# Farama-Foundation/Gymnasium-Robotics

Measured on NVIDIA H100. Metric: env-steps/s, higher is better.
Workload: dtype f32

## Files before the change

### gymnasium_robotics_b200/csrc/sim_core.cuh

```cuda
#pragma once
#include "dmodel.h"

#if defined(__CUDACC__) || defined(B200_HOST_WARP)
#define B200_WARP_CODE 1
#endif
#ifdef __CUDACC__
#define HD static __device__ __forceinline__
#define HDN static __device__ __noinline__
#define STAGE static __device__ __noinline__
#define ASSUME_SHARED_PTR(p) __builtin_assume(__isShared(p))
#define ASSUME_SHARED(c) do { __builtin_assume(__isShared((c).s)); __builtin_assume(__isShared((c).mw)); __builtin_assume(__isShared((c).h)); } while (0)
#define WARP_W 32
#define SYNC() __syncwarp()
#define ALIGN() __syncthreads()
#define ALIGN_OR(p) __syncthreads_or(p)
#elif defined(B200_HOST_WARP)
#define HD static inline
#define HDN static
#define STAGE static
#define ASSUME_SHARED(c) do { } while (0)
#define ASSUME_SHARED_PTR(p) do { } while (0)
#define WARP_W 32
#define SYNC() __syncwarp()
#define ALIGN() __syncwarp()
#define ALIGN_OR(p) (__ballot_sync(0xffffffffu, (p)) != 0u)
static inline float rsqrtf(float x) { return 1.0f / sqrtf(x); }
#else
#define HD static inline
#define HDN static
#define STAGE static
#define ASSUME_SHARED(c) do { } while (0)
#define ASSUME_SHARED_PTR(p) do { } while (0)
#define WARP_W 1
#define SYNC() do { } while (0)
#define ALIGN() do { } while (0)
#define ALIGN_OR(p) (p)
static inline float rsqrtf(float x) { return 1.0f / sqrtf(x); }
#endif

#define B200_MINVAL 1e-15f
#define B200_MINIMP 0.0001f
#define B200_MAXIMP 0.9999f

struct Ctx {
  const uint32_t* mg;
  const uint32_t* mw;
  const DMHead* h;
  float* s;
  int lane;
#ifdef B200_STAGE_TIMING
  long long* tim;
#endif
};
#ifdef B200_STAGE_TIMING
enum { TM_KIN = 0, TM_COM_M, TM_COLL, TM_CONSTR, TM_SMOOTH, TM_NBEGIN, TM_NCHECK, TM_BUILDH, TM_NDIR, TM_NMOVE, TM_INTEG, TM_BARRIER, TM_OTHER, TM_MV_MULM, TM_MV_ROWS, TM_MV_LS, TM_CK_PASSF, TM_MV_UPD, TM_COUNT };
#define TIC() long long t0_ = clock64()
#define TOC(k) do { long long t1_ = clock64(); c.tim[k] += t1_ - t0_; t0_ = t1_; } while (0)
#else
#define TIC() do { } while (0)
#define TOC(k) do { } while (0)
#endif
#ifdef __CUDACC__
extern __shared__ __align__(128) uint32_t b200_smem[];
#endif
template <bool REBUILD>
HD Ctx stage_ctx(const Ctx& c) {
#ifdef __CUDACC__
  if (REBUILD) {
    uint32_t tid;
    asm volatile("mov.u32 %0, %%tid.x;" : "=r"(tid));
    Ctx r = c;
    const DMHead* h = (const DMHead*)b200_smem;
    r.s = (float*)(b200_smem + h->hot_words) + (tid >> 5) * h->scr_words;
    r.lane = (int)(tid & 31);
    return r;
  }
#endif
  return c;
}
#define MI(name) ((const int*)(c.mw + c.h->o_##name))
#define MU(name) ((const uint32_t*)(c.mw + c.h->o_##name))
#define MF(name) ((const float*)(c.mw + c.h->o_##name))
#ifdef B200_KITCHEN_GROUPS
#define PAIR_I(name) ((const int*)(c.mg + c.h->o_##name))
#define PAIR_F(name) ((const float*)(c.mg + c.h->o_##name))
#else
#define PAIR_I(name) MI(name)
#define PAIR_F(name) MF(name)
#endif
#define GI(name) ((const int*)(c.mg + c.h->o_##name))
#define GF(name) ((const float*)(c.mg + c.h->o_##name))
#define SF(name) (c.s + c.h->s_##name)
#define SI(name) ((int*)(c.s + c.h->s_##name))
#define LANES(i, n) for (int i = c.lane; i < (n); i += WARP_W)

HD float wsum(float v) {
#ifdef B200_WARP_CODE
  for (int o = 16; o; o >>= 1) v += __shfl_xor_sync(0xffffffffu, v, o);
#endif
  return v;
}
HD float wmax(float v) {
#ifdef B200_WARP_CODE
  for (int o = 16; o; o >>= 1) v = fmaxf(v, __shfl_xor_sync(0xffffffffu, v, o));
#endif
  return v;
}
HD int wsumi(int v) {
#ifdef B200_WARP_CODE
  for (int o = 16; o; o >>= 1) v += __shfl_xor_sync(0xffffffffu, v, o);
#endif
  return v;
}
HD int wexscan(int v, int lane, int* total) {
#ifdef B200_WARP_CODE
  int x = v;
  for (int o = 1; o < 32; o <<= 1) { int y = __shfl_up_sync(0xffffffffu, x, o); if (lane >= o) x += y; }
  *total = __shfl_sync(0xffffffffu, x, 31);
  return x - v;
#else
  (void)lane; *total = v; return 0;
#endif
}
HD int ffs_pop(uint32_t& m) {
#ifdef __CUDACC__
  int b = __ffs(m) - 1;
#else
  int b = __builtin_ctz(m);
#endif
  m &= m - 1;
  return b;
}
#ifdef B200_WIDE
typedef unsigned long long dmask_t;
HD int ffs_pop(dmask_t& m) {
#ifdef __CUDACC__
  int b = __ffsll((long long)m) - 1;
#else
  int b = __builtin_ctzll(m);
#endif
  m &= m - 1;
  return b;
}
// ... 1118 lines not shown
      if (id >= h->ncon_max) break;
      float* cr = SF(con) + id * CON_WORDS;
      cr[0] = o.pos[k][0]; cr[1] = o.pos[k][1]; cr[2] = o.pos[k][2];
      cr[3] = o.nrm[k][0]; cr[4] = o.nrm[k][1]; cr[5] = o.nrm[k][2];
      cr[6] = o.dist[k];
      ((int*)cr)[7] = p;
      ((int*)cr)[C_DIMGRP] = gid << 8;
      kept++;
    }
    if (ocnt > 0) {
      int* gi = (int*)(SF(group) + gid * GRP_WORDS);
      int ba = MI(geom_body)[PAIR_I(pair_geom1)[p]], bb = PAIR_I(pair_geom2)[p] < 0 ? 0 : MI(geom_body)[PAIR_I(pair_geom2)[p]];
      dmask_t ma = DM(body_ancdof, ba), mb = DM(body_ancdof, bb);
      const int bodies = GI(geom_mjb)[PAIR_I(pair_geom1)[p]] | ((PAIR_I(pair_geom2)[p] < 0 ? 0 : GI(geom_mjb)[PAIR_I(pair_geom2)[p]]) << 8);
      ((uint32_t*)gi)[G_RANGE] = (uint32_t)(basec + slot) | (uint32_t)kept << 8 | (uint32_t)bodies << 16;
      grp_set_masks(gi, ma ^ mb, mb);
    }
    if (c.lane == 0) {
      int nn = basec + total; if (nn > h->ncon_max) { nn = h->ncon_max; cnt[CNT_OVERFLOW] |= 2; }
      int ng = baseg + gtotal; if (ng > h->ngrp_max - DM_NWELD_MAX) { ng = h->ngrp_max - DM_NWELD_MAX; cnt[CNT_OVERFLOW] |= 4; }
      cnt[CNT_NCON] = nn; cnt[CNT_NGRP] = ng;
    }
    SYNC();
  }
  LANES(id, cnt[CNT_NCON]) {
    float* cr = SF(con) + id * CON_WORDS;
    const float pos[3] = {cr[0], cr[1], cr[2]}, dist = cr[6];
    float fr9[9] = {cr[3], cr[4], cr[5], 0, 0, 0, 0, 0, 0};
    const int p = ((const int*)cr)[7], gid8 = ((const int*)cr)[C_DIMGRP];
    make_frame(fr9);
    float r[3] = {pos[0] - h->ref[0], pos[1] - h->ref[1], pos[2] - h->ref[2]};
    for (int a = 0; a < 3; a++) { float* w = cr + C_W + 6 * a; cross3(w, r, fr9 + 3 * a); w[3] = fr9[3 * a]; w[4] = fr9[3 * a + 1]; w[5] = fr9[3 * a + 2]; }
    const float* fr = GF(pair_friction) + 3 * p;
    int dim = GI(pair_condim)[p];
    float mu0 = fr[0];
    cr[C_MU] = mu0; cr[C_MU + 1] = fr[1];
#ifdef B200_KITCHEN
    cr[C_MU + 2] = fr[2];
#endif
    float incl = PAIR_F(pair_margin)[p] - GF(pair_gap)[p];
    float solimp[5] = {GF(pair_solimp)[5 * p], GF(pair_solimp)[5 * p + 1], GF(pair_solimp)[5 * p + 2], GF(pair_solimp)[5 * p + 3], GF(pair_solimp)[5 * p + 4]};
    float solref[2] = {GF(pair_solref)[2 * p], GF(pair_solref)[2 * p + 1]};
    float imp = impedance(solimp, dist, incl);
    float K, Bc;
    ref_kb(c, solref, solimp[1], &K, &Bc);
    float tran = GF(pair_invweight)[2 * p];
    float R;
    if (dim == 1) R = fmaxf((1 - imp) / imp * tran, B200_MINVAL);
    else {
      float R0 = fmaxf((1 - imp) / imp * (tran + mu0 * mu0 * tran), B200_MINVAL);
      float mu = mu0 * rsqrtf(h->impratio);
      R = fmaxf(2 * mu * mu * R0, B200_MINVAL);
    }
    cr[C_D] = 1.0f / R;
    cr[C_U] = K * imp * (dist - incl); cr[C_U + 1] = 0; cr[C_U + 2] = 0; cr[C_U + 3] = 0;
#ifdef B200_KITCHEN
    cr[C_U + 4] = 0; cr[C_U + 5] = 0;
#endif
    cr[C_JV] = Bc;
    ((int*)cr)[C_DIMGRP] = dim | gid8;
    if (HF && h->nsensor > 0) {
      float* cx = SF(conx) + id * CX_WORDS;
      cx[CX_POS] = pos[0]; cx[CX_POS + 1] = pos[1]; cx[CX_POS + 2] = pos[2];
      ((int*)cx)[CX_PAIR] = p;
    }
  }
  SYNC();
}

#ifdef B200_KITCHEN
HD void con_w(const float* cr, int k, float* w) {
  if (k < 3) { const float* s = cr + C_W + 6 * k; w[0] = s[0]; w[1] = s[1]; w[2] = s[2]; w[3] = s[3]; w[4] = s[4]; w[5] = s[5]; }
  else { const float* s = cr + C_W + 6 * (k - 3) + 3; w[0] = s[0]; w[1] = s[1]; w[2] = s[2]; w[3] = w[4] = w[5] = 0; }
}
HD float con_mu(const float* cr, int k) { return k < 3 ? cr[C_MU] : (k == 3 ? cr[C_MU + 1] : cr[C_MU + 2]); }
#else
HD void con_w(const float* cr, int k, float* w) {
  if (k < 3) { const float* s = cr + C_W + 6 * k; w[0] = s[0]; w[1] = s[1]; w[2] = s[2]; w[3] = s[3]; w[4] = s[4]; w[5] = s[5]; }
  else { w[0] = cr[C_W + 3]; w[1] = cr[C_W + 4]; w[2] = cr[C_W + 5]; w[3] = w[4] = w[5] = 0; }
}
HD float con_mu(const float* cr, int k) { return k < 3 ? cr[C_MU] : cr[C_MU + 1]; }
#endif
HD int con_dim(const float* cr) { return ((const int*)cr)[C_DIMGRP] & 0xff; }
HD int con_grp(const float* cr) { return ((const int*)cr)[C_DIMGRP] >> 8; }

template <bool HF>
STAGE void make_constraint(const Ctx c) {
  ASSUME_SHARED(c);
  const DMHead* h = c.h;
  int* cnt = SI(counters);
  if (c.lane == 0) { cnt[CNT_NDR] = 0; cnt[CNT_NWELD] = 0; }
  SYNC();
  for (int e = 0; e < h->neq; e++) {
    if (!MI(eq_active)[e] || MI(eq_type)[e] != B200_EQ_WELD) continue;
    const int nw = cnt[CNT_NWELD], gid = cnt[CNT_NGRP];
    float* wr = SF(weld) + nw * WELD_WORDS;
    const float* data = MF(eq_data) + 11 * e;
    int s1 = MI(eq_obj1)[e], s2 = MI(eq_obj2)[e], b1 = 0, b2 = 0;
    float p1[3] = {0, 0, 0}, p2[3] = {0, 0, 0}, q1[4] = {1, 0, 0, 0}, q2[4] = {1, 0, 0, 0}, t[3];
    if (s1 >= 0) { b1 = MI(site_body)[s1]; qmul(q1, SF(xquat) + 4 * b1, MF(site_quat) + 4 * s1); qrot(t, SF(xquat) + 4 * b1, MF(site_pos) + 3 * s1); for (int k = 0; k < 3; k++) p1[k] = SF(xpos)[3 * b1 + k] + t[k]; }
    if (s2 >= 0) { b2 = MI(site_body)[s2]; qmul(q2, SF(xquat) + 4 * b2, MF(site_quat) + 4 * s2); qrot(t, SF(xquat) + 4 * b2, MF(site_pos) + 3 * s2); for (int k = 0; k < 3; k++) p2[k] = SF(xpos)[3 * b2 + k] + t[k]; }
    qrot(t, q1, data + 3); for (int k = 0; k < 3; k++) p1[k] += t[k];
    qrot(t, q2, data + 0); for (int k = 0; k < 3; k++) p2[k] += t[k];
    const float ts = data[10];
    float quat[4], quat1[4] = {q2[0], -q2[1], -q2[2], -q2[3]}, quat2[4];
    qmul(quat, q1, data + 6);
    qmul(quat2, quat1, quat);
    const bool use1 = b1 > 0 && DM(body_ancdof, b1) != 0;
    float r[3];
    for (int k = 0; k < 3; k++) r[k] = (use1 ? p1[k] : p2[k]) - h->ref[k];
    float K, Bc;
    ref_kb(c, MF(eq_solref) + 2 * e, MF(eq_solimp)[5 * e + 1], &K, &Bc);
    LANES(k, 6) {
      float* w = wr + W_W + 6 * k;
      float cp;
      if (k < 3) {
        float e3[3] = {k == 0 ? 1.f : 0.f, k == 1 ? 1.f : 0.f, k == 2 ? 1.f : 0.f};
        cross3(w, r, e3); w[3] = e3[0]; w[4] = e3[1]; w[5] = e3[2];
        cp = k == 0 ? p1[0] - p2[0] : (k == 1 ? p1[1] - p2[1] : p1[2] - p2[2]);
      } else {
        const int kk = k - 3;
        for (int a = 0; a < 3; a++) {
          float qa[4] = {0, a == 0 ? 1.f : 0.f, a == 1 ? 1.f : 0.f, a == 2 ? 1.f : 0.f}, t1[4], t2[4];
          qmul(t1, quat1, qa); qmul(t2, t1, quat);
          w[a] = 0.5f * ts * (kk == 0 ? t2[1] : (kk == 1 ? t2[2] : t2[3])); w[3 + a] = 0;
        }
        cp = ts * (kk == 0 ? quat2[1] : (kk == 1 ? quat2[2] : quat2[3]));
      }
      float imp = impedance(MF(eq_solimp) + 5 * e, cp, 0.f);
      float R = fmaxf((1 - imp) / imp * MF(eq_invweight)[2 * e + (k < 3 ? 0 : 1)], B200_MINVAL);
      wr[W_D + k] = 1.0f / R; wr[W_JAR + k] = K * imp * cp;
    }
    if (c.lane == 0) {
      wr[W_B] = Bc;
      ((int*)wr)[W_GRP] = gid;
      int* gi = (int*)(SF(group) + gid * GRP_WORDS);
      dmask_t ma = DM(body_ancdof, b2), mb = DM(body_ancdof, b1);
      gi[G_RANGE] = 0;
      grp_set_masks(gi, ma ^ mb, mb);
    }
    SYNC();
    if (c.lane == 0) { cnt[CNT_NGRP] = gid + 1; cnt[CNT_NWELD] = nw + 1; }
    SYNC();
  }
  for (int base = 0; base < h->njnt; base += WARP_W) {
    int j = base + c.lane;
    int nrow = 0; float dist0 = 0, dist1 = 0, sgn0 = 0, sgn1 = 0;
    if (j < h->njnt && MI(jnt_limited)[j] && MI(jnt_type)[j] != B200_JNT_FREE) {
      float q = SF(qpos)[MI(jnt_qposadr)[j]], margin = MF(jnt_margin)[j];
      float dl = q - MF(jnt_range)[2 * j], du = MF(jnt_range)[2 * j + 1] - q;
      if (dl < margin) { dist0 = dl; sgn0 = 1.f; nrow = 1; }
      if (du < margin) { if (nrow) { dist1 = du; sgn1 = -1.f; } else { dist0 = du; sgn0 = -1.f; } nrow++; }
    }
    int total, slot = wexscan(nrow, c.lane, &total);
    int basec = cnt[CNT_NDR];
    SYNC();
#pragma unroll
    for (int k = 0; k < 2; k++) {
      int id = basec + slot + k;
      if (k >= nrow || id >= h->ndr_max) continue;
      const float distk = k ? dist1 : dist0, sgnk = k ? sgn1 : sgn0;
      float* dr = SF(dofrow) + id * DR_WORDS;
      int* di = (int*)dr;
      int d = MI(jnt_dofadr)[j];
      float margin = MF(jnt_margin)[j];
      float solimp[5] = {GF(jnt_solimp)[5 * j], GF(jnt_solimp)[5 * j + 1], GF(jnt_solimp)[5 * j + 2], GF(jnt_solimp)[5 * j + 3], GF(jnt_solimp)[5 * j + 4]};
      float solref[2] = {GF(jnt_solref)[2 * j], GF(jnt_solref)[2 * j + 1]};
      float imp = impedance(solimp, distk, margin);
      float K, Bc;
      ref_kb(c, solref, solimp[1], &K, &Bc);
      float R = fmaxf((1 - imp) / imp * MF(dof_invweight0)[d], B200_MINVAL);
      di[DR_DOF] = d; dr[DR_COEF] = sgnk; di[DR_DOF2] = -1; dr[DR_COEF2] = 0;
      dr[DR_D] = 1.0f / R; dr[DR_JAR] = K * imp * (distk - margin); dr[DR_JV] = Bc;
    }
    if (c.lane == 0) { int nn = basec + total; if (nn > h->ndr_max) { nn = h->ndr_max; cnt[CNT_OVERFLOW] |= 8; } cnt[CNT_NDR] = nn; }
    SYNC();
  }
  if (HF) for (int base = 0; base < h->nten; base += WARP_W) {
    int t = base + c.lane;
    int nrow = 0; float dist0 = 0, dist1 = 0, sgn0 = 0, sgn1 = 0;
    if (t < h->nten) {
      float len = MF(ten_coef)[2 * t] * SF(qpos)[MI(ten_qadr)[2 * t]];
      if (MI(ten_dof)[2 * t + 1] >= 0) len += MF(ten_coef)[2 * t + 1] * SF(qpos)[MI(ten_qadr)[2 * t + 1]];
      float margin = MF(ten_margin)[t];
      float dl = len - MF(ten_range)[2 * t], du = MF(ten_range)[2 * t + 1] - len;
      if (dl < margin) { dist0 = dl; sgn0 = 1.f; nrow = 1; }
      if (du < margin) { if (nrow) { dist1 = du; sgn1 = -1.f; } else { dist0 = du; sgn0 = -1.f; } nrow++; }
    }
    int total, slot = wexscan(nrow, c.lane, &total);
    int basec = cnt[CNT_NDR];
    SYNC();
#pragma unroll
    for (int k = 0; k < 2; k++) {
      int id = basec + slot + k;
      if (k >= nrow || id >= h->ndr_max) continue;
      const float distk = k ? dist1 : dist0, sgnk = k ? sgn1 : sgn0;
      float* dr = SF(dofrow) + id * DR_WORDS;
      int* di = (int*)dr;
      float margin = MF(ten_margin)[t];
      float solimp[5] = {GF(ten_solimp)[5 * t], GF(ten_solimp)[5 * t + 1], GF(ten_solimp)[5 * t + 2], GF(ten_solimp)[5 * t + 3], GF(ten_solimp)[5 * t + 4]};
      float solref[2] = {GF(ten_solref)[2 * t], GF(ten_solref)[2 * t + 1]};
      float imp = impedance(solimp, distk, margin);
      float K, Bc;
      ref_kb(c, solref, solimp[1], &K, &Bc);
      float R = fmaxf((1 - imp) / imp * GF(ten_invweight)[t], B200_MINVAL);
      di[DR_DOF] = MI(ten_dof)[2 * t]; dr[DR_COEF] = sgnk * MF(ten_coef)[2 * t];
      di[DR_DOF2] = MI(ten_dof)[2 * t + 1]; dr[DR_COEF2] = sgnk * MF(ten_coef)[2 * t + 1];
      dr[DR_D] = 1.0f / R; dr[DR_JAR] = K * imp * (distk - margin); dr[DR_JV] = Bc;
    }
    if (c.lane == 0) { int nn = basec + total; if (nn > h->ndr_max) { nn = h->ndr_max; cnt[CNT_OVERFLOW] |= 8; } cnt[CNT_NDR] = nn; }
    SYNC();
  }
#ifdef B200_KITCHEN
  if (c.lane == 0) {
    for (int e = 0; e < h->neq; e++) {
      if (!MI(eq_active)[e] || MI(eq_type)[e] != B200_EQ_JOINT) continue;
      int id = cnt[CNT_NDR];
      if (id >= h->ndr_max) { cnt[CNT_OVERFLOW] |= 8; break; }
      const float* data = MF(eq_data) + 11 * e;
      int j1 = MI(eq_obj1)[e], j2 = MI(eq_obj2)[e];
      float pos = SF(qpos)[MI(jnt_qposadr)[j1]] - MF(jnt_qpos0)[j1], deriv = 0.f;
      if (j2 >= 0) {
        float dif = SF(qpos)[MI(jnt_qposadr)[j2]] - MF(jnt_qpos0)[j2];
        pos -= data[0] + dif * (data[1] + dif * (data[2] + dif * (data[3] + dif * data[4])));
        deriv = data[1] + dif * (2 * data[2] + dif * (3 * data[3] + dif * 4 * data[4]));
      } else pos -= data[0];
      float* dr = SF(dofrow) + id * DR_WORDS;
      int* di = (int*)dr;
      float imp = impedance(MF(eq_solimp) + 5 * e, pos, 0.f);
      float K, Bc;
      ref_kb(c, MF(eq_solref) + 2 * e, MF(eq_solimp)[5 * e + 1], &K, &Bc);
      float R = fmaxf((1 - imp) / imp * MF(eq_invweight)[2 * e], B200_MINVAL);
      di[DR_DOF] = MI(jnt_dofadr)[j1]; dr[DR_COEF] = 1.f;
      di[DR_DOF2] = j2 >= 0 ? MI(jnt_dofadr)[j2] : -1; dr[DR_COEF2] = -deriv;
      dr[DR_D] = -1.0f / R; dr[DR_JAR] = K * imp * pos; dr[DR_JV] = Bc;
      cnt[CNT_NDR] = id + 1;
    }
  }
  SYNC();
#endif
  if (HF) { LANES(d, h->nfric) SF(fric)[d] = 0.f; SYNC(); }
}

template <bool HF>
STAGE void rows_from_vec(const Ctx c, const float* vec) {
  ASSUME_SHARED(c);
  ASSUME_SHARED_PTR(vec);
  const int* cnt = SI(counters);
  int ngrp = cnt[CNT_NGRP];
  LANES(idx, ngrp * 6) {
    int g = idx / 6, a = idx - 6 * g;
    float* gr = SF(group) + g * GRP_WORDS;
    dmask_t S = grp_mask(gr), sg = grp_sign(gr);
    float acc = 0;
    while (S) { int j = ffs_pop(S); float t = SF(cdof)[6 * j + a] * vec[j]; acc += DBIT(sg, j) ? t : -t; }
    gr[G_V + a] = acc;
  }
  SYNC();
  LANES(i, cnt[CNT_NCON]) {
    float* cr = SF(con) + i * CON_WORDS;
    int dim = con_dim(cr), nbase = dim == 1 ? 1 : dim;
    const float* dV = SF(group) + con_grp(cr) * GRP_WORDS + G_V;
    for (int k = 0; k < nbase; k++) {
      float w[6];
      con_w(cr, k, w);
      cr[C_JV + k] = dot6(w, dV);
    }
  }
  LANES(i, cnt[CNT_NWELD] * 6) {
    float* wr = SF(weld) + (i / 6) * WELD_WORDS;
    int k = i % 6;
    const float* dV = SF(group) + ((const int*)wr)[W_GRP] * GRP_WORDS + G_V;
    wr[W_JV + k] = dot6(wr + W_W + 6 * k, dV);
  }
  LANES(i, cnt[CNT_NDR]) {
    float* dr = SF(dofrow) + i * DR_WORDS;
    const int* di = (const int*)dr;
    float val = dr[DR_COEF] * vec[di[DR_DOF]];
    if (di[DR_DOF2] >= 0) val += dr[DR_COEF2] * vec[di[DR_DOF2]];
    dr[DR_JV] = val;
  }
  if (HF) LANES(d, c.h->nfric) SF(fric)[c.h->nfric + d] = vec[d];
  SYNC();
}

template <bool HF>
STAGE void rows_begin(const Ctx c, const float* qvel, const float* qacc) {
  ASSUME_SHARED(c);
  ASSUME_SHARED_PTR(qvel); ASSUME_SHARED_PTR(qacc);
  const int* cnt = SI(counters);
  int ngrp = cnt[CNT_NGRP];
  float* dA = SF(H);
  LANES(idx, ngrp * 6) {
    int g = idx / 6, a = idx - 6 * g;
    float* gr = SF(group) + g * GRP_WORDS;
    dmask_t S = grp_mask(gr), sg = grp_sign(gr);
    float acc = 0, acc2 = 0;
    while (S) {
      int j = ffs_pop(S);
      float cd = SF(cdof)[6 * j + a], t = cd * qvel[j], t2 = cd * qacc[j];
      bool pos = DBIT(sg, j);
      acc += pos ? t : -t; acc2 += pos ? t2 : -t2;
    }
    gr[G_V + a] = acc; dA[idx] = acc2;
  }
  SYNC();
  LANES(i, cnt[CNT_NCON]) {
    float* cr = SF(con) + i * CON_WORDS;
    int dim = con_dim(cr), nbase = dim == 1 ? 1 : dim;
    const float* gr = SF(group) + con_grp(cr) * GRP_WORDS;
    const float* gA = dA + 6 * con_grp(cr);
    float Bc = cr[C_JV];
    for (int k = 0; k < nbase; k++) {
      float w[6];
      con_w(cr, k, w);
      float u = cr[C_U + k];
      u += Bc * dot6(w, gr + G_V);
      u += dot6(w, gA);
      cr[C_U + k] = u;
    }
  }
  LANES(i, cnt[CNT_NWELD] * 6) {
    float* wr = SF(weld) + (i / 6) * WELD_WORDS;
    int k = i % 6;
    const int g = ((const int*)wr)[W_GRP];
    const float* gr = SF(group) + g * GRP_WORDS;
    float u = wr[W_JAR + k];
    u += wr[W_B] * dot6(wr + W_W + 6 * k, gr + G_V);
    u += dot6(wr + W_W + 6 * k, dA + 6 * g);
    wr[W_JAR + k] = u;
  }
  LANES(i, cnt[CNT_NDR]) {
    float* dr = SF(dofrow) + i * DR_WORDS;
    const int* di = (const int*)dr;
    float v1 = dr[DR_COEF] * qvel[di[DR_DOF]], v2 = dr[DR_COEF] * qacc[di[DR_DOF]];
    if (di[DR_DOF2] >= 0) { v1 += dr[DR_COEF2] * qvel[di[DR_DOF2]]; v2 += dr[DR_COEF2] * qacc[di[DR_DOF2]]; }
    float u = dr[DR_JAR];
    u += dr[DR_JV] * v1;
    u += v2;
    dr[DR_JAR] = u;
  }
  if (HF) LANES(d, c.h->nfric) {
    float* fr = SF(fric);
    float u = fr[d];
    u += MF(dof_fricB)[d] * qvel[d];
    u += qacc[d];
    fr[d] = u;
  }
  SYNC();
}

HD void contact_base_forces(const float* cr, int dim, float* F) {
  float D = cr[C_D], un = cr[C_U];
#pragma unroll
  for (int k = 0; k < C_NB; k++) F[k] = 0;
  if (dim == 1) { F[0] = un < 0 ? -D * un : 0.f; return; }
#pragma unroll
  for (int k = 1; k < C_NB; k++) {
    if (k >= dim) continue;
    float mu = con_mu(cr, k), uk = cr[C_U + k];
    float xp = un + mu * uk, xm = un - mu * uk;
    float fp = xp < 0 ? -D * xp : 0.f, fm = xm < 0 ? -D * xm : 0.f;
    F[0] += fp + fm;
    F[k] = mu * (fp - fm);
  }
}

template <bool HF>
STAGE void pass_F(const Ctx c, float* out) {
  ASSUME_SHARED(c);
  ASSUME_SHARED_PTR(out);
  const DMHead* h = c.h;
  const int* cnt = SI(counters);
  int ngrp = cnt[CNT_NGRP], nweld = cnt[CNT_NWELD], ndr = cnt[CNT_NDR];
  LANES(i, cnt[CNT_NCON]) {
    float* cr = SF(con) + i * CON_WORDS;
    float F[C_NB];
    contact_base_forces(cr, con_dim(cr), F);
    cr[C_JV] = F[0]; cr[C_JV + 1] = F[1]; cr[C_JV + 2] = F[2]; cr[C_JV + 3] = F[3];
#ifdef B200_KITCHEN
    cr[C_JV + 4] = F[4]; cr[C_JV + 5] = F[5];
#endif
  }
  SYNC();
  LANES(idx, ngrp * 6) {
    int g = idx / 6, a = idx - 6 * g;
    float* gr = SF(group) + g * GRP_WORDS;
    float acc = 0;
    for (int i = grp_start(gr), i1 = i + grp_count(gr); i < i1; i++) {
      const float* cr = SF(con) + i * CON_WORDS;
      int dim = con_dim(cr);
      const float* F = cr + C_JV;
      acc += F[0] * cr[C_W + a];
      if (dim > 1) acc += F[1] * cr[C_W + 6 + a] + F[2] * cr[C_W + 12 + a];
      if (dim > 3 && a < 3) acc += F[3] * cr[C_W + 3 + a];
#ifdef B200_KITCHEN
      if (dim > 4 && a < 3) acc += F[4] * cr[C_W + 6 + 3 + a] + F[5] * cr[C_W + 12 + 3 + a];
#endif
    }
    for (int i = 0; i < nweld; i++) {
      const float* wr = SF(weld) + i * WELD_WORDS;
      if (((const int*)wr)[W_GRP] != g) continue;
      for (int k = 0; k < 6; k++) acc -= wr[W_D + k] * wr[W_JAR + k] * wr[W_W + 6 * k + a];
    }
    gr[G_V + a] = acc;
  }
  SYNC();
  LANES(j, h->nv) {
    float q = 0;
    const float* cd = SF(cdof) + 6 * j;
    for (int g = 0; g < ngrp; g++) {
      const float* gr = SF(group) + g * GRP_WORDS;
      if (!DBIT(grp_mask(gr), j)) continue;
      float d = dot6(cd, gr + G_V);
      q += DBIT(grp_sign(gr), j) ? d : -d;
    }
    for (int i = 0; i < ndr; i++) {
      const float* dr = SF(dofrow) + i * DR_WORDS;
      const int* di = (const int*)dr;
      float x = dr[DR_JAR];
#ifdef B200_KITCHEN
      float f = (dr[DR_D] < 0 || x < 0) ? -fabsf(dr[DR_D]) * x : 0.f;
#else
      float f = x < 0 ? -dr[DR_D] * x : 0.f;
#endif
      if (di[DR_DOF] == j) q += dr[DR_COEF] * f;
      if (di[DR_DOF2] == j) q += dr[DR_COEF2] * f;
    }
    if (HF && h->nfric) {
      float fl = MF(dof_frictionloss)[j];
      q += fminf(fmaxf(-MF(dof_fricD)[j] * SF(fric)[j], -fl), fl);
    }
    out[j] = q;
  }
  SYNC();
}

STAGE void mulM(const Ctx c, const float* v, float* out) {
  ASSUME_SHARED(c);
  ASSUME_SHARED_PTR(v); ASSUME_SHARED_PTR(out);
  int nv = c.h->nv;
  const float* M = SF(M);
  LANES(i, nv) {
    float a = 0;
    const int row = i * (i + 1) / 2;
    for (int j = 0; j <= i; j++) a += M[row + j] * v[j];
    for (int j = i + 1, idx = row + 2 * i + 1; j < nv; idx += ++j) a += M[idx] * v[j];
    out[i] = a;
  }
  SYNC();
}

template <bool HF>
STAGE void build_H(const Ctx c) {
  ASSUME_SHARED(c);
  const DMHead* h = c.h;
  const int* cnt = SI(counters);
  int nv = h->nv, nM = nv * (nv + 1) / 2, nweld = cnt[CNT_NWELD], ngrp = cnt[CNT_NGRP], ndr = cnt[CNT_NDR];
  float* H = SF(H);
  LANES(i, nM) H[i] = SF(M)[i];
  float* Kc = H + nM;
  const int kcap = (h->s_grad - h->s_H - nM) / 21;
  for (int g0 = 0; g0 < ngrp; g0 += kcap) {
    const int g1 = ngrp - g0 < kcap ? ngrp : g0 + kcap;
    LANES(e, 21) {
      int r = 0; while ((r + 1) * (r + 2) / 2 <= e) r++;
      const int s = e - r * (r + 1) / 2;
      for (int g = g0; g < g1; g++) {
        float* K = Kc + 21 * (g - g0);
        const float* gr = SF(group) + g * GRP_WORDS;
        float acc = 0;
        for (int i = grp_start(gr), i1 = i + grp_count(gr); i < i1; i++) {
          const float* cr = SF(con) + i * CON_WORDS;
          int dim = con_dim(cr);
          float D = cr[C_D], un = cr[C_U];
          float wnr = cr[C_W + r], wns = cr[C_W + s];
          if (dim == 1) { if (un < 0) acc += D * wnr * wns; continue; }
          float Wnn = 0;
          for (int k = 1; k < dim; k++) {
            float mu = con_mu(cr, k), uk = cr[C_U + k];
            float ap = (un + mu * uk) < 0 ? 1.f : 0.f, am = (un - mu * uk) < 0 ? 1.f : 0.f;
            if (ap + am == 0.f) continue;
            float wkr, wks;
            if (k < 3) { wkr = cr[C_W + 6 * k + r]; wks = cr[C_W + 6 * k + s]; }
#ifdef B200_KITCHEN
            else { wkr = r < 3 ? cr[C_W + 6 * (k - 3) + 3 + r] : 0.f; wks = s < 3 ? cr[C_W + 6 * (k - 3) + 3 + s] : 0.f; }
#else
            else { wkr = r < 3 ? cr[C_W + 3 + r] : 0.f; wks = s < 3 ? cr[C_W + 3 + s] : 0.f; }
#endif
            Wnn += ap + am;
            float Wnk = mu * (ap - am), Wkk = mu * mu * (ap + am);
            acc += D * (Wnk * (wnr * wks + wkr * wns) + Wkk * wkr * wks);
          }
          acc += D * Wnn * wnr * wns;
        }
        for (int i = 0; i < nweld; i++) {
          const float* wr = SF(weld) + i * WELD_WORDS;
          if (((const int*)wr)[W_GRP] != g) continue;
          for (int k = 0; k < 6; k++) acc += wr[W_D + k] * wr[W_W + 6 * k + r] * wr[W_W + 6 * k + s];
        }
        K[e] = acc;
      }
    }
    SYNC();
    LANES(i, nv) {
      const float* cd = SF(cdof) + 6 * i;
      const int row = i * (i + 1) / 2;
      for (int g = g0; g < g1; g++) {
        const float* gr = SF(group) + g * GRP_WORDS;
        const dmask_t S = grp_mask(gr), mb = grp_sign(gr);
        if (!DBIT(S, i)) continue;
        const float* K = Kc + 21 * (g - g0);
        float y[6];
#pragma unroll
        for (int r = 0; r < 6; r++) {
          float a = 0;
#pragma unroll
          for (int s2 = 0; s2 < 6; s2++) a += K[pidx(r, s2)] * cd[s2];
          y[r] = a;
        }
        float si = DBIT(mb, i) ? 1.f : -1.f;
        dmask_t m2 = S & (((dmask_t)2 << i) - (dmask_t)1);
        while (m2) {
          int j = ffs_pop(m2);
          float sj = DBIT(mb, j) ? 1.f : -1.f;
          H[row + j] += si * sj * dot6(SF(cdof) + 6 * j, y);
        }
      }
    }
    SYNC();
  }
  SYNC();
  if (HF) {
    LANES(d, h->nfric) {
      float D = MF(dof_fricD)[d], x = SF(fric)[d];
      if (D > 0 && fabsf(x) * D < MF(dof_frictionloss)[d]) H[d * (d + 1) / 2 + d] += D;
    }
    SYNC();
  }
  if (HF) {
    LANES(j, nv) {
      float diag = 0.f;
      for (int i = 0; i < ndr; i++) {
        const float* dr = SF(dofrow) + i * DR_WORDS;
        const int* di = (const int*)dr;
#ifdef B200_KITCHEN
        if (!(dr[DR_JAR] < 0 || dr[DR_D] < 0)) continue;
        const float Dr = fabsf(dr[DR_D]);
#else
        if (!(dr[DR_JAR] < 0)) continue;
        const float& Dr = dr[DR_D];
#endif
        int d1 = di[DR_DOF], d2 = di[DR_DOF2];
        if (d1 == j) diag += Dr * dr[DR_COEF] * dr[DR_COEF];
        if (d2 == j) diag += Dr * dr[DR_COEF2] * dr[DR_COEF2];
        if (d2 >= 0 && (d1 > d2 ? d1 : d2) == j) H[j * (j + 1) / 2 + (d1 > d2 ? d2 : d1)] += Dr * dr[DR_COEF] * dr[DR_COEF2];
      }
      H[j * (j + 1) / 2 + j] += diag;
    }
  } else if (c.lane == 0) {
    for (int i = 0; i < ndr; i++) {
      const float* dr = SF(dofrow) + i * DR_WORDS;
      const int* di = (const int*)dr;
      if (!(dr[DR_JAR] < 0)) continue;
      int d1 = di[DR_DOF], d2 = di[DR_DOF2];
// ... 282 lines not shown
STAGE int ls_edges(const Ctx c) {
  ASSUME_SHARED(c);
  const DMHead* h = c.h;
  const int* cnt = SI(counters);
  const int epc = h->edges_per_con, ncon = cnt[CNT_NCON], nweld6 = cnt[CNT_NWELD] * 6, ndr = cnt[CNT_NDR];
  float* E = SF(H);
  LANES(i, ncon) {
    const float* cr = SF(con) + i * CON_WORDS;
    float* e = E + 3 * epc * i;
    int dim = con_dim(cr);
    float D = cr[C_D], un = cr[C_U], vn = cr[C_JV];
    int ne = 0;
    if (dim == 1) { e[0] = un; e[1] = vn; e[2] = D; ne = 1; }
    else for (int k = 1; k < dim; k++) {
      float mu = con_mu(cr, k), uk = mu * cr[C_U + k], vk = mu * cr[C_JV + k];
      e[3 * ne] = un + uk; e[3 * ne + 1] = vn + vk; e[3 * ne + 2] = D; ne++;
      e[3 * ne] = un - uk; e[3 * ne + 1] = vn - vk; e[3 * ne + 2] = D; ne++;
    }
    for (; ne < epc; ne++) e[3 * ne + 2] = 0.f;
  }
  float* W = E + 3 * epc * ncon;
  LANES(i, nweld6) {
    const float* wr = SF(weld) + (i / 6) * WELD_WORDS;
    int k = i % 6;
    W[3 * i] = wr[W_JAR + k]; W[3 * i + 1] = wr[W_JV + k]; W[3 * i + 2] = -wr[W_D + k];
  }
  float* R = W + 3 * nweld6;
  LANES(i, ndr) {
    const float* dr = SF(dofrow) + i * DR_WORDS;
    R[3 * i] = dr[DR_JAR]; R[3 * i + 1] = dr[DR_JV]; R[3 * i + 2] = dr[DR_D];
  }
  SYNC();
  return epc * ncon + nweld6 + ndr;
}

template <bool HF>
STAGE void ls_eval(const Ctx c, int nedge, float alpha, float g1, float g2, float* out) {
  ASSUME_SHARED(c);
  float cost = 0, d1 = 0, d2 = 0;
  const float* E = SF(H);
  LANES(i, nedge) {
    float x0 = E[3 * i], v = E[3 * i + 1], D = E[3 * i + 2];
    float x = fmaf(alpha, v, x0), Da = fabsf(D);
    if (D < 0 || (x < 0 && D > 0)) { float dx = Da * x; cost = fmaf(0.5f * dx, x, cost); d1 = fmaf(dx, v, d1); d2 = fmaf(Da * v, v, d2); }
  }
  if (HF) LANES(d, c.h->nfric) {
    float D = MF(dof_fricD)[d];
    if (D > 0) {
      float fl = MF(dof_frictionloss)[d], v = SF(fric)[c.h->nfric + d], x = SF(fric)[d] + alpha * v, Rf = fl / D;
      if (x <= -Rf) { cost += fl * (-0.5f * Rf - x); d1 -= fl * v; }
      else if (x >= Rf) { cost += fl * (-0.5f * Rf + x); d1 += fl * v; }
      else { cost += 0.5f * D * x * x; d1 += D * x * v; d2 += D * v * v; }
    }
  }
  out[0] = wsum(cost) + alpha * g1 + alpha * alpha * g2;
  out[1] = wsum(d1) + g1 + 2 * alpha * g2;
  out[2] = wsum(d2) + 2 * g2;
}

template <bool HF, int LSE>
STAGE LsStep linesearch(const Ctx c, float g1, float g2, float gtol, int maxit) {
  ASSUME_SHARED(c);
  float p0[3], p[3];
  const int nedge = ls_edges<HF>(c);
  ls_eval<HF>(c, nedge, 0.f, g1, g2, p0);
  if (p0[1] >= 0 || p0[2] <= 0) return LsStep{0.f, 0.f};
  gtol = fmaxf(gtol, 1e-5f * fabsf(p0[1]));
  float lo = 0, hi = -1, alpha = -p0[1] / p0[2], best = 0, bestcost = p0[0];
  for (int it = 0; it < maxit; it++) {
    ls_eval<HF>(c, nedge, alpha, g1, g2, p);
    if (p[0] <= bestcost) { bestcost = p[0]; best = alpha; }
    if (fabsf(p[1]) < gtol) break;
    if (p[1] < 0) lo = alpha; else hi = alpha;
    float next = alpha - p[1] / p[2];
    if (hi > 0 && (next <= lo || next >= hi)) next = 0.5f * (lo + hi);
    if (next == alpha) break;
    alpha = next;
  }
  return LsStep{best, p0[0] - bestcost};
}

#endif

template <bool HF>
STAGE void newton_begin(const Ctx c) {
  ASSUME_SHARED(c);
  mulM(c, SF(qacc), SF(Ma));
  rows_begin<HF>(c, SF(qvel), SF(qacc));
}

template <bool HF>
STAGE int newton_check(const Ctx c, int iter, float improvement) {
  ASSUME_SHARED(c);
  const DMHead* h = c.h;
  int nv = h->nv;
  float *Ma = SF(Ma), *grad = SF(grad), *fs = SF(fsmooth), *fcon = SF(fcon);
  float scale = 1.0f / (h->meaninertia * (float)(nv > 1 ? nv : 1));
  float tol = fmaxf(h->tolerance, 1e-6f);
  TIC();
  pass_F<HF>(c, fcon);
  TOC(TM_CK_PASSF);
  float g2sum = 0, f2sum = 0;
  LANES(i, nv) {
    float g = Ma[i] - fs[i] - fcon[i], f = fabsf(Ma[i]) + fabsf(fs[i]) + fabsf(fcon[i]);
    grad[i] = g; g2sum += g * g; f2sum += f * f;
  }
  SYNC();
  float gnorm = sqrtf(wsum(g2sum)), fnorm = sqrtf(wsum(f2sum));
  if (gnorm < 2e-6f * fnorm) return 1;
  if (iter > 0 && (scale * improvement < tol || scale * gnorm < tol)) return 1;
  if (iter >= h->iterations || iter >= 12) return 1;
  return 0;
}

template <int NVP>
STAGE void newton_direction(const Ctx c) {
  ASSUME_SHARED(c);
  int nv = c.h->nv;
  LANES(i, nv) SF(search)[i] = -SF(grad)[i];
  SYNC();
  spd_solve<NVP>(c, SF(H), nullptr, 0.f, SF(search), SF(H));
}

template <bool HF, int LSE>
STAGE int newton_move(const Ctx c, float* improvement) {
  ASSUME_SHARED(c);
  const DMHead* h = c.h;
  int nv = h->nv;
  int* cnt = SI(counters);
  float *a = SF(qacc), *Ma = SF(Ma), *Mv = SF(Mv), *search = SF(search), *fs = SF(fsmooth);
  float scale = 1.0f / (h->meaninertia * (float)(nv > 1 ? nv : 1));
  TIC();
  mulM(c, search, Mv);
  TOC(TM_MV_MULM);
  rows_from_vec<HF>(c, search);
  TOC(TM_MV_ROWS);
  float q1 = 0, q2 = 0, sn = 0;
  LANES(i, nv) { q1 += search[i] * (Ma[i] - fs[i]); q2 += 0.5f * search[i] * Mv[i]; sn += search[i] * search[i]; }
  q1 = wsum(q1); q2 = wsum(q2); sn = sqrtf(wsum(sn));
  if (sn < 1e-20f) return 1;
  float gtol = h->tolerance * h->ls_tolerance * sn / scale;
  TOC(TM_MV_ROWS);
  const LsStep ls = linesearch<HF, LSE>(c, q1, q2, gtol, h->ls_iterations < 20 ? h->ls_iterations : 20);
  *improvement = ls.improve;
  const float alpha = ls.alpha;
  TOC(TM_MV_LS);
  if (alpha == 0.f) return 1;
  LANES(i, nv) { a[i] += alpha * search[i]; Ma[i] += alpha * Mv[i]; }
  LANES(i, cnt[CNT_NCON]) { float* cr = SF(con) + i * CON_WORDS; for (int k = 0; k < C_NB; k++) cr[C_U + k] += alpha * cr[C_JV + k]; }
  LANES(i, cnt[CNT_NWELD] * 6) { float* wr = SF(weld) + (i / 6) * WELD_WORDS; wr[W_JAR + i % 6] += alpha * wr[W_JV + i % 6]; }
  LANES(i, cnt[CNT_NDR]) { float* dr = SF(dofrow) + i * DR_WORDS; dr[DR_JAR] += alpha * dr[DR_JV]; }
  if (HF) LANES(d, h->nfric) SF(fric)[d] += alpha * SF(fric)[h->nfric + d];
  SYNC();
  if (c.lane == 0) cnt[CNT_ITERS] += 1;
  TOC(TM_MV_UPD);
  return 0;
}

template <int NVP>
STAGE void euler_solve(const Ctx c) {
  ASSUME_SHARED(c);
  const DMHead* h = c.h;
  float* x = SF(search);
  LANES(i, h->nv) x[i] = SF(fsmooth)[i] + SF(fcon)[i];
  SYNC();
  spd_solve<NVP>(c, SF(M), MF(dof_damping), h->timestep, x, SF(H));
}

template <int NVP, bool REBUILD = false>
HD void forward(const Ctx c, bool active) {
  constexpr bool HF = NVP >= 30;
  constexpr bool CX = NVP == 22 || NVP >= 30;
  constexpr int kLsE = DM_LS_E(NVP);
  TIC();
  ALIGN(); TOC(TM_BARRIER);
  if (active) kinematics(stage_ctx<REBUILD>(c));
  TOC(TM_KIN); if (HF) ALIGN(); TOC(TM_BARRIER);
  if (active) { com_quantities(stage_ctx<REBUILD>(c)); mass_matrix(stage_ctx<REBUILD>(c)); }
  TOC(TM_COM_M); ALIGN(); TOC(TM_BARRIER);
  if (active) collision<HF, CX>(stage_ctx<REBUILD>(c));
  TOC(TM_COLL); ALIGN(); TOC(TM_BARRIER);
  if (active) make_constraint<HF>(stage_ctx<REBUILD>(c));
  TOC(TM_CONSTR); if (HF) ALIGN(); TOC(TM_BARRIER);
  if (active) smooth_forces(stage_ctx<REBUILD>(c));
  TOC(TM_SMOOTH); if (HF) ALIGN(); TOC(TM_BARRIER);
  if (active) newton_begin<HF>(stage_ctx<REBUILD>(c));
  TOC(TM_NBEGIN);
  int done = active ? 0 : 1;
  float improvement = 0;
  for (int iter = 0;; iter++) {
    ALIGN(); TOC(TM_BARRIER);
    if (!done) done = newton_check<HF>(stage_ctx<REBUILD>(c), iter, improvement);
    TOC(TM_NCHECK);
    bool more = ALIGN_OR(!done);
    TOC(TM_BARRIER);
    if (!more) break;
    if (!done) build_H<HF>(stage_ctx<REBUILD>(c));
    TOC(TM_BUILDH); if (HF) ALIGN(); TOC(TM_BARRIER);
    if (!done) newton_direction<NVP>(stage_ctx<REBUILD>(c));
    TOC(TM_NDIR); ALIGN(); TOC(TM_BARRIER);
    if (!done) done = newton_move<HF, kLsE>(stage_ctx<REBUILD>(c), &improvement) ? 2 : 0;
    TOC(TM_NMOVE);
  }
}

STAGE void integrate_pos(const Ctx c, float* qpos, const float* qvel, float hh) {
  ASSUME_SHARED(c);
  ASSUME_SHARED_PTR(qpos); ASSUME_SHARED_PTR(qvel);
  const DMHead* h = c.h;
  LANES(j, h->njnt) {
    int a = MI(jnt_qposadr)[j], d = MI(jnt_dofadr)[j];
    if (MI(jnt_type)[j] == B200_JNT_FREE) {
      for (int k = 0; k < 3; k++) qpos[a + k] += hh * qvel[d + k];
      float w[3] = {qvel[d + 3], qvel[d + 4], qvel[d + 5]};
      float n = sqrtf(dot3(w, w));
      float q[4] = {qpos[a + 3], qpos[a + 4], qpos[a + 5], qpos[a + 6]};
      if (n > 0) {
        float ang = 0.5f * n * hh, sn = sinf(ang), cs = cosf(ang), inv = 1.0f / n;
        float dq[4] = {cs, w[0] * inv * sn, w[1] * inv * sn, w[2] * inv * sn}, nq[4];
        qmul(nq, q, dq);
        q[0] = nq[0]; q[1] = nq[1]; q[2] = nq[2]; q[3] = nq[3];
      }
      qnormalize(q);
      qpos[a + 3] = q[0]; qpos[a + 4] = q[1]; qpos[a + 5] = q[2]; qpos[a + 6] = q[3];
    } else qpos[a] += hh * qvel[d];
  }
  SYNC();
}

template <int NVP>
STAGE void euler_step(const Ctx c) {
  ASSUME_SHARED(c);
  const DMHead* h = c.h;
  int nv = h->nv;
  float hh = h->timestep;
  float* x = SF(search);
  if (h->any_damping) {
    euler_solve<NVP>(c);
  } else {
    LANES(i, nv) x[i] = SF(qacc)[i];
    SYNC();
  }
  LANES(i, nv) SF(qvel)[i] += hh * x[i];
  SYNC();
  integrate_pos(c, SF(qpos), SF(qvel), hh);
}

template <int NVP, bool REBUILD = false>
HD void rk4_substep(const Ctx c, bool active) {
  const DMHead* h = c.h;
  const int nv = h->nv, nq = h->nq;
  const float hh = h->timestep;
  const float A[3] = {0.5f, 0.5f, 1.0f}, B[4] = {1.0f / 6, 1.0f / 3, 1.0f / 3, 1.0f / 6};
  if (active) {
    LANES(i, nq) SF(rk_q0)[i] = SF(qpos)[i];
    LANES(i, nv) { SF(rk_v0)[i] = SF(qvel)[i]; SF(rk_dx)[i] = B[0] * SF(qvel)[i]; SF(rk_df)[i] = B[0] * SF(qacc)[i]; }
    SYNC();
  }
  for (int st = 1; st < 4; st++) {
    if (active) {
      float a = A[st - 1] * hh;
      LANES(i, nq) SF(qpos)[i] = SF(rk_q0)[i];
      SYNC();
      integrate_pos(c, SF(qpos), SF(qvel), a);
      LANES(i, nv) SF(qvel)[i] = SF(rk_v0)[i] + a * SF(qacc)[i];
      SYNC();
    }
    forward<NVP, REBUILD>(c, active);
    if (active) {
      LANES(i, nv) { SF(rk_dx)[i] += B[st] * SF(qvel)[i]; SF(rk_df)[i] += B[st] * SF(qacc)[i]; }
      SYNC();
    }
  }
  if (active) {
    LANES(i, nq) SF(qpos)[i] = SF(rk_q0)[i];
    LANES(i, nv) SF(qvel)[i] = SF(rk_v0)[i] + hh * SF(rk_df)[i];
    SYNC();
    integrate_pos(c, SF(qpos), SF(rk_dx), hh);
  }
}
```

Baseline: 1.093 million.

## Cache contact activity bits and fuse Newton check into begin/move stages

Contact forces and their active-cone bitmask are now computed inline whenever constraint velocities U are updated, in rows_begin and in the newton_move update. The bitmask is packed into the dim/group word, so pass_F and build_H no longer recompute forces or the activity tests. newton_check is folded into newton_begin and newton_move, which removes one block barrier per iteration, and some ALIGN barriers are skipped when REBUILD is set. The group field is now masked to 8 bits, which caps the number of groups, and skipping barriers in REBUILD mode relies on each warp working only on its own scratch.

```diff
diff --git a/gymnasium_robotics_b200/csrc/sim_core.cuh b/gymnasium_robotics_b200/csrc/sim_core.cuh
--- a/gymnasium_robotics_b200/csrc/sim_core.cuh
+++ b/gymnasium_robotics_b200/csrc/sim_core.cuh
@@ -56,9 +56,13 @@
 enum { TM_KIN = 0, TM_COM_M, TM_COLL, TM_CONSTR, TM_SMOOTH, TM_NBEGIN, TM_NCHECK, TM_BUILDH, TM_NDIR, TM_NMOVE, TM_INTEG, TM_BARRIER, TM_OTHER, TM_MV_MULM, TM_MV_ROWS, TM_MV_LS, TM_CK_PASSF, TM_MV_UPD, TM_COUNT };
 #define TIC() long long t0_ = clock64()
 #define TOC(k) do { long long t1_ = clock64(); c.tim[k] += t1_ - t0_; t0_ = t1_; } while (0)
+#define CHECK_TIC() long long tc_ = clock64()
+#define CHECK_TOC(stage) do { long long d_ = clock64() - tc_; c.tim[TM_NCHECK] += d_; c.tim[stage] -= d_; } while (0)
 #else
 #define TIC() do { } while (0)
 #define TOC(k) do { } while (0)
+#define CHECK_TIC() do { } while (0)
+#define CHECK_TOC(stage) do { } while (0)
 #endif
 #ifdef __CUDACC__
 extern __shared__ __align__(128) uint32_t b200_smem[];
@@ -1343,7 +1347,8 @@
 HD float con_mu(const float* cr, int k) { return k < 3 ? cr[C_MU] : cr[C_MU + 1]; }
 #endif
 HD int con_dim(const float* cr) { return ((const int*)cr)[C_DIMGRP] & 0xff; }
-HD int con_grp(const float* cr) { return ((const int*)cr)[C_DIMGRP] >> 8; }
+HD int con_grp(const float* cr) { return (((const int*)cr)[C_DIMGRP] >> 8) & 0xff; }
+HD uint32_t con_act(const float* cr) { return ((const uint32_t*)cr)[C_DIMGRP] >> 16; }
 
 template <bool HF>
 STAGE void make_constraint(const Ctx c) {
@@ -1503,6 +1508,39 @@
   if (HF) { LANES(d, h->nfric) SF(fric)[d] = 0.f; SYNC(); }
 }
 
+HD uint32_t contact_base_forces(const float* cr, int dim, const float (&U)[C_NB], float* F) {
+  float D = cr[C_D], un = U[0];
+#pragma unroll
+  for (int k = 0; k < C_NB; k++) F[k] = 0;
+  if (dim == 1) { F[0] = un < 0 ? -D * un : 0.f; return un < 0 ? 1u : 0u; }
+  uint32_t act = 0;
+#pragma unroll
+  for (int k = 1; k < C_NB; k++) {
+    if (k >= dim) continue;
+    float mu = con_mu(cr, k), uk = U[k];
+    float xp = un + mu * uk, xm = un - mu * uk;
+    float fp = xp < 0 ? -D * xp : 0.f, fm = xm < 0 ? -D * xm : 0.f;
+    act |= (xp < 0 ? 1u : 0u) << (2 * k - 2) | (xm < 0 ? 1u : 0u) << (2 * k - 1);
+    F[0] += fp + fm;
+    F[k] = mu * (fp - fm);
+  }
+  return act;
+}
+HD void contact_base_forces(const float* cr, int dim, float* F) {
+  float U[C_NB];
+#pragma unroll
+  for (int k = 0; k < C_NB; k++) U[k] = cr[C_U + k];
+  contact_base_forces(cr, dim, U, F);
+}
+HD void contact_park_forces(float* cr, const float (&U)[C_NB]) {
+  int* dg = (int*)cr + C_DIMGRP;
+  float F[C_NB];
+  const uint32_t act = contact_base_forces(cr, *dg & 0xff, U, F);
+#pragma unroll
+  for (int k = 0; k < C_NB; k++) cr[C_JV + k] = F[k];
+  *dg = (int)(((uint32_t)*dg & 0xffffu) | act << 16);
+}
+
 template <bool HF>
 STAGE void rows_from_vec(const Ctx c, const float* vec) {
   ASSUME_SHARED(c);
@@ -1572,14 +1610,20 @@
     const float* gr = SF(group) + con_grp(cr) * GRP_WORDS;
     const float* gA = dA + 6 * con_grp(cr);
     float Bc = cr[C_JV];
-    for (int k = 0; k < nbase; k++) {
+    float U[C_NB];
+#pragma unroll
+    for (int k = 0; k < C_NB; k++) {
+      U[k] = 0.f;
+      if (k >= nbase) continue;
       float w[6];
       con_w(cr, k, w);
       float u = cr[C_U + k];
       u += Bc * dot6(w, gr + G_V);
       u += dot6(w, gA);
       cr[C_U + k] = u;
-    }
+      U[k] = u;
+    }
+    contact_park_forces(cr, U);
   }
   LANES(i, cnt[CNT_NWELD] * 6) {
     float* wr = SF(weld) + (i / 6) * WELD_WORDS;
@@ -1611,39 +1655,12 @@
   SYNC();
 }
 
-HD void contact_base_forces(const float* cr, int dim, float* F) {
-  float D = cr[C_D], un = cr[C_U];
-#pragma unroll
-  for (int k = 0; k < C_NB; k++) F[k] = 0;
-  if (dim == 1) { F[0] = un < 0 ? -D * un : 0.f; return; }
-#pragma unroll
-  for (int k = 1; k < C_NB; k++) {
-    if (k >= dim) continue;
-    float mu = con_mu(cr, k), uk = cr[C_U + k];
-    float xp = un + mu * uk, xm = un - mu * uk;
-    float fp = xp < 0 ? -D * xp : 0.f, fm = xm < 0 ? -D * xm : 0.f;
-    F[0] += fp + fm;
-    F[k] = mu * (fp - fm);
-  }
-}
-
 template <bool HF>
-STAGE void pass_F(const Ctx c, float* out) {
-  ASSUME_SHARED(c);
-  ASSUME_SHARED_PTR(out);
+HD void pass_F(const Ctx c, float* out) {
+  ASSUME_SHARED(c);
   const DMHead* h = c.h;
   const int* cnt = SI(counters);
   int ngrp = cnt[CNT_NGRP], nweld = cnt[CNT_NWELD], ndr = cnt[CNT_NDR];
-  LANES(i, cnt[CNT_NCON]) {
-    float* cr = SF(con) + i * CON_WORDS;
-    float F[C_NB];
-    contact_base_forces(cr, con_dim(cr), F);
-    cr[C_JV] = F[0]; cr[C_JV + 1] = F[1]; cr[C_JV + 2] = F[2]; cr[C_JV + 3] = F[3];
-#ifdef B200_KITCHEN
-    cr[C_JV + 4] = F[4]; cr[C_JV + 5] = F[5];
-#endif
-  }
-  SYNC();
   LANES(idx, ngrp * 6) {
     int g = idx / 6, a = idx - 6 * g;
     float* gr = SF(group) + g * GRP_WORDS;
@@ -1733,15 +1750,16 @@
         float acc = 0;
         for (int i = grp_start(gr), i1 = i + grp_count(gr); i < i1; i++) {
           const float* cr = SF(con) + i * CON_WORDS;
-          int dim = con_dim(cr);
-          float D = cr[C_D], un = cr[C_U];
+          const int dim = con_dim(cr);
+          const uint32_t act = con_act(cr);
+          float D = cr[C_D];
           float wnr = cr[C_W + r], wns = cr[C_W + s];
-          if (dim == 1) { if (un < 0) acc += D * wnr * wns; continue; }
+          if (dim == 1) { if (act & 1u) acc += D * wnr * wns; continue; }
           float Wnn = 0;
           for (int k = 1; k < dim; k++) {
-            float mu = con_mu(cr, k), uk = cr[C_U + k];
-            float ap = (un + mu * uk) < 0 ? 1.f : 0.f, am = (un - mu * uk) < 0 ? 1.f : 0.f;
+            float ap = (act >> (2 * k - 2)) & 1u ? 1.f : 0.f, am = (act >> (2 * k - 1)) & 1u ? 1.f : 0.f;
             if (ap + am == 0.f) continue;
+            float mu = con_mu(cr, k);
             float wkr, wks;
             if (k < 3) { wkr = cr[C_W + 6 * k + r]; wks = cr[C_W + 6 * k + s]; }
 #ifdef B200_KITCHEN
@@ -2190,15 +2208,9 @@
 
 #endif
 
+
 template <bool HF>
-STAGE void newton_begin(const Ctx c) {
-  ASSUME_SHARED(c);
-  mulM(c, SF(qacc), SF(Ma));
-  rows_begin<HF>(c, SF(qvel), SF(qacc));
-}
-
-template <bool HF>
-STAGE int newton_check(const Ctx c, int iter, float improvement) {
+HD int newton_check(const Ctx c, int iter, float improvement) {
   ASSUME_SHARED(c);
   const DMHead* h = c.h;
   int nv = h->nv;
@@ -2221,6 +2233,17 @@
   return 0;
 }
 
+template <bool HF>
+STAGE int newton_begin(const Ctx c) {
+  ASSUME_SHARED(c);
+  mulM(c, SF(qacc), SF(Ma));
+  rows_begin<HF>(c, SF(qvel), SF(qacc));
+  CHECK_TIC();
+  const int done = newton_check<HF>(c, 0, 0.f);
+  CHECK_TOC(TM_NBEGIN);
+  return done;
+}
+
 template <int NVP>
 STAGE void newton_direction(const Ctx c) {
   ASSUME_SHARED(c);
@@ -2231,7 +2254,7 @@
 }
 
 template <bool HF, int LSE>
-STAGE int newton_move(const Ctx c, float* improvement) {
+STAGE int newton_move(const Ctx c, int iter) {
   ASSUME_SHARED(c);
   const DMHead* h = c.h;
   int nv = h->nv;
@@ -2246,23 +2269,31 @@
   float q1 = 0, q2 = 0, sn = 0;
   LANES(i, nv) { q1 += search[i] * (Ma[i] - fs[i]); q2 += 0.5f * search[i] * Mv[i]; sn += search[i] * search[i]; }
   q1 = wsum(q1); q2 = wsum(q2); sn = sqrtf(wsum(sn));
-  if (sn < 1e-20f) return 1;
+  if (sn < 1e-20f) return 2;
   float gtol = h->tolerance * h->ls_tolerance * sn / scale;
   TOC(TM_MV_ROWS);
   const LsStep ls = linesearch<HF, LSE>(c, q1, q2, gtol, h->ls_iterations < 20 ? h->ls_iterations : 20);
-  *improvement = ls.improve;
   const float alpha = ls.alpha;
   TOC(TM_MV_LS);
-  if (alpha == 0.f) return 1;
+  if (alpha == 0.f) return 2;
   LANES(i, nv) { a[i] += alpha * search[i]; Ma[i] += alpha * Mv[i]; }
-  LANES(i, cnt[CNT_NCON]) { float* cr = SF(con) + i * CON_WORDS; for (int k = 0; k < C_NB; k++) cr[C_U + k] += alpha * cr[C_JV + k]; }
+  LANES(i, cnt[CNT_NCON]) {
+    float* cr = SF(con) + i * CON_WORDS;
+    float U[C_NB];
+#pragma unroll
+    for (int k = 0; k < C_NB; k++) { U[k] = cr[C_U + k] + alpha * cr[C_JV + k]; cr[C_U + k] = U[k]; }
+    contact_park_forces(cr, U);
+  }
   LANES(i, cnt[CNT_NWELD] * 6) { float* wr = SF(weld) + (i / 6) * WELD_WORDS; wr[W_JAR + i % 6] += alpha * wr[W_JV + i % 6]; }
   LANES(i, cnt[CNT_NDR]) { float* dr = SF(dofrow) + i * DR_WORDS; dr[DR_JAR] += alpha * dr[DR_JV]; }
   if (HF) LANES(d, h->nfric) SF(fric)[d] += alpha * SF(fric)[h->nfric + d];
   SYNC();
   if (c.lane == 0) cnt[CNT_ITERS] += 1;
   TOC(TM_MV_UPD);
-  return 0;
+  CHECK_TIC();
+  const int done = newton_check<HF>(c, iter + 1, ls.improve);
+  CHECK_TOC(TM_NMOVE);
+  return done;
 }
 
 template <int NVP>
@@ -2287,27 +2318,23 @@
   if (active) { com_quantities(stage_ctx<REBUILD>(c)); mass_matrix(stage_ctx<REBUILD>(c)); }
   TOC(TM_COM_M); ALIGN(); TOC(TM_BARRIER);
   if (active) collision<HF, CX>(stage_ctx<REBUILD>(c));
-  TOC(TM_COLL); ALIGN(); TOC(TM_BARRIER);
+  TOC(TM_COLL); if (!REBUILD) ALIGN(); TOC(TM_BARRIER);
   if (active) make_constraint<HF>(stage_ctx<REBUILD>(c));
   TOC(TM_CONSTR); if (HF) ALIGN(); TOC(TM_BARRIER);
   if (active) smooth_forces(stage_ctx<REBUILD>(c));
   TOC(TM_SMOOTH); if (HF) ALIGN(); TOC(TM_BARRIER);
-  if (active) newton_begin<HF>(stage_ctx<REBUILD>(c));
+  int done = 1;
+  if (active) done = newton_begin<HF>(stage_ctx<REBUILD>(c));
   TOC(TM_NBEGIN);
-  int done = active ? 0 : 1;
-  float improvement = 0;
   for (int iter = 0;; iter++) {
-    ALIGN(); TOC(TM_BARRIER);
-    if (!done) done = newton_check<HF>(stage_ctx<REBUILD>(c), iter, improvement);
-    TOC(TM_NCHECK);
     bool more = ALIGN_OR(!done);
     TOC(TM_BARRIER);
     if (!more) break;
     if (!done) build_H<HF>(stage_ctx<REBUILD>(c));
     TOC(TM_BUILDH); if (HF) ALIGN(); TOC(TM_BARRIER);
     if (!done) newton_direction<NVP>(stage_ctx<REBUILD>(c));
-    TOC(TM_NDIR); ALIGN(); TOC(TM_BARRIER);
-    if (!done) done = newton_move<HF, kLsE>(stage_ctx<REBUILD>(c), &improvement) ? 2 : 0;
+    TOC(TM_NDIR); if (!REBUILD) ALIGN(); TOC(TM_BARRIER);
+    if (!done) done = newton_move<HF, kLsE>(stage_ctx<REBUILD>(c), iter);
     TOC(TM_NMOVE);
   }
 }
```

New measurement: 1.140 million, median of 6. 1.04x the previous value.
